# xuekt98/BBDM

Measured on NVIDIA H100. Metric: denoising-steps/sec (UNet fwd) at 256^2 pixel-BBDM, higher is better.
Workload: dtype bf16x3 (split-bf16 tensor-core products, fp32 accumulate: fp32-class)

## Files before the change

### bbdm_b200/csrc/conv_umma.cu

```cuda
#include "tc_common.cuh"
#include <stdlib.h>

namespace bbdm {

constexpr int UM_BM = 128;
constexpr int UM_BK = 64;
constexpr int UM_THREADS = 384;
constexpr int UM_PRODUCER_REGS = 40, UM_CONSUMER_REGS = 232;
static_assert(128 * UM_PRODUCER_REGS + 256 * UM_CONSUMER_REGS <= 65536, "conv_umma: register split");
constexpr int UM_SLICES = 4;

struct ConvParams {
  int B, H, W, Cout;
  int TW, TH, TB, tiles_w, tiles_h, tiles_b, n_tiles;
  int kb_per_tap;
  int K1;
  int K2;
  int taps;
  int up2;
  int origin;
  int w_per_image;
  int kb_per_chunk;
  const float* bias; const float* bias2;
  const float* residual; int res_mode;
  float* out; __nv_bfloat16* out_hi; __nv_bfloat16* out_lo;
  int out_nchw_c;
  float* stats;
  unsigned long long* fault;
};

template <int BN>
struct UmmaCfg {
  static constexpr uint32_t A_BYTES = UM_BM * UM_BK * 2;
  static constexpr uint32_t W_BYTES = BN * UM_BK * 2;
  static constexpr uint32_t STAGE3 = 2 * A_BYTES + 2 * W_BYTES;
  static constexpr uint32_t STAGE1 = A_BYTES + W_BYTES;
  static constexpr uint32_t SMEM_BUDGET = 200 * 1024;
  static constexpr int STAGES3 = (SMEM_BUDGET / STAGE3) > 6 ? 6 : (SMEM_BUDGET / STAGE3);
  static constexpr int STAGES1 = (SMEM_BUDGET / STAGE1) > 8 ? 8 : (SMEM_BUDGET / STAGE1);
};

template <int BN, bool F16>
__device__ __forceinline__ void conv_mma(float* d, uint64_t da, uint64_t db) {
  if (F16) {
    if (BN == 128) wgmma_n128_f16<0>(d, da, db, 1u); else wgmma_n64_f16<0>(d, da, db, 1u);
  } else {
    if (BN == 128) wgmma_n128_bf16<0>(d, da, db, 1u); else wgmma_n64_bf16<0>(d, da, db, 1u);
  }
}

struct EpiTile {
  int nb, tw, th, tb, phase;
  int bb[2], hh[2], ww[2];
  bool valid[2];
  int64_t pix[2];
};

__device__ __forceinline__ EpiTile epi_tile(const ConvParams& p, int tile, int n_blocks, int warp, int lane) {
  EpiTile e;
  e.nb = tile % n_blocks;
  int mt = tile / n_blocks;
  e.phase = 0;
  if (p.up2) { e.phase = mt & 3; mt >>= 2; }
  e.tw = mt % p.tiles_w; mt /= p.tiles_w;
  e.th = mt % p.tiles_h;
  e.tb = mt / p.tiles_h;
  const int OH = p.up2 ? 2 * p.H : p.H, OW = p.up2 ? 2 * p.W : p.W;
#pragma unroll
  for (int ri = 0; ri < 2; ++ri) {
    const int row = 16 * warp + (lane >> 2) + 8 * ri;
    const int ws = e.tw * p.TW + row % p.TW;
    const int hs = e.th * p.TH + (row / p.TW) % p.TH;
    e.bb[ri] = e.tb * p.TB + row / (p.TW * p.TH);
    e.valid[ri] = ws < p.W && hs < p.H && e.bb[ri] < p.B;
    e.hh[ri] = p.up2 ? 2 * hs + (e.phase >> 1) : hs;
    e.ww[ri] = p.up2 ? 2 * ws + (e.phase & 1) : ws;
    e.pix[ri] = ((int64_t)e.bb[ri] * OH + e.hh[ri]) * OW + e.ww[ri];
  }
  return e;
}

template <int BN>
__device__ __forceinline__ void epi_slice(const ConvParams& p, const float* racc, EpiTile e, int s, int warp,
                                          int lane, float (*stats_s)[BN][2]) {
  constexpr int JS = BN / 8 / UM_SLICES;
  if (e.nb * BN + s * (BN / UM_SLICES) >= p.Cout) return;
  asm volatile("" : "+r"(e.nb), "+r"(e.bb[0]), "+r"(e.bb[1]), "+r"(e.hh[0]), "+r"(e.hh[1]), "+r"(e.ww[0]),
               "+r"(e.ww[1]), "+l"(e.pix[0]), "+l"(e.pix[1]));
  const int OH = p.up2 ? 2 * p.H : p.H, OW = p.up2 ? 2 * p.W : p.W;
  const int n0 = e.nb * BN + 2 * (lane & 3);
  float2 v[2][JS];
#pragma unroll
  for (int ri = 0; ri < 2; ++ri) {
#pragma unroll
    for (int j = 0; j < JS; ++j) {
      const int jj = JS * s + j;
      const int nc = n0 + 8 * jj;
      v[ri][j] = make_float2(racc[4 * jj + 2 * ri], racc[4 * jj + 2 * ri + 1]);
      if (p.bias) { const float2 b = *reinterpret_cast<const float2*>(p.bias + nc); v[ri][j].x += b.x; v[ri][j].y += b.y; }
      if (p.bias2) { const float2 b = *reinterpret_cast<const float2*>(p.bias2 + nc); v[ri][j].x += b.x; v[ri][j].y += b.y; }
    }
  }
  if (p.res_mode == BBDM_RES_SAME || p.res_mode == BBDM_RES_UP2) {
#pragma unroll
    for (int ri = 0; ri < 2; ++ri) {
      if (!e.valid[ri]) continue;
      const int64_t rpix = p.res_mode == BBDM_RES_SAME
                               ? e.pix[ri]
                               : ((int64_t)e.bb[ri] * (OH >> 1) + (e.hh[ri] >> 1)) * (OW >> 1) + (e.ww[ri] >> 1);
      const float* rp = p.residual + rpix * p.Cout + n0 + 8 * JS * s;
#pragma unroll
      for (int j = 0; j < JS; ++j) {
        const float2 t = *reinterpret_cast<const float2*>(rp + 8 * j);
        v[ri][j].x += t.x; v[ri][j].y += t.y;
      }
    }
  } else if (p.res_mode == BBDM_RES_DOWN2) {
    const int64_t W2 = (int64_t)OW * 2;
#pragma unroll
    for (int ri = 0; ri < 2; ++ri) {
      if (!e.valid[ri]) continue;
      const float* rp0 = p.residual + (((int64_t)e.bb[ri] * OH * 2 + e.hh[ri] * 2) * W2 + e.ww[ri] * 2) * p.Cout +
                         n0 + 8 * JS * s;
#pragma unroll
      for (int j = 0; j < JS; ++j) {
        const float* rp = rp0 + 8 * j;
        const float2 t0 = *reinterpret_cast<const float2*>(rp), t1 = *reinterpret_cast<const float2*>(rp + p.Cout);
        const float2 t2 = *reinterpret_cast<const float2*>(rp + W2 * p.Cout);
        const float2 t3 = *reinterpret_cast<const float2*>(rp + (W2 + 1) * p.Cout);
        v[ri][j].x += 0.25f * (((t0.x + t1.x) + t2.x) + t3.x);
        v[ri][j].y += 0.25f * (((t0.y + t1.y) + t2.y) + t3.y);
      }
    }
  }
  float ssum[2 * JS], ssq[2 * JS];
#pragma unroll
  for (int j = 0; j < 2 * JS; ++j) { ssum[j] = 0.f; ssq[j] = 0.f; }
#pragma unroll
  for (int ri = 0; ri < 2; ++ri) {
    if (!e.valid[ri]) continue;
    const int bb = e.bb[ri], hh = e.hh[ri], ww = e.ww[ri];
    const int64_t pix = e.pix[ri];
#pragma unroll
    for (int j = 0; j < JS; ++j) {
      const int nc = n0 + 8 * (JS * s + j);
      const float2 w = v[ri][j];
      if (p.out_nchw_c > 0) {
        if (nc < p.out_nchw_c) p.out[(((int64_t)bb * p.out_nchw_c + nc) * OH + hh) * OW + ww] = w.x;
        if (nc + 1 < p.out_nchw_c) p.out[(((int64_t)bb * p.out_nchw_c + nc + 1) * OH + hh) * OW + ww] = w.y;
      } else if (p.out) {
        *reinterpret_cast<float2*>(p.out + pix * p.Cout + nc) = w;
      }
      if (p.out_hi) {
        uint32_t h, l;
        split2x(w.x, w.y, h, l);
        *reinterpret_cast<uint32_t*>(p.out_hi + pix * p.Cout + nc) = h;
        *reinterpret_cast<uint32_t*>(p.out_lo + pix * p.Cout + nc) = l;
      }
      ssum[2 * j] += w.x; ssq[2 * j] += w.x * w.x;
      ssum[2 * j + 1] += w.y; ssq[2 * j + 1] += w.y * w.y;
    }
  }
  if (p.stats) {
#pragma unroll
    for (int j = 0; j < 2 * JS; ++j) {
#pragma unroll
      for (int off = 4; off < 32; off <<= 1) {
        ssum[j] += __shfl_xor_sync(0xffffffffu, ssum[j], off);
        ssq[j] += __shfl_xor_sync(0xffffffffu, ssq[j], off);
      }
    }
    if (lane < 4) {
#pragma unroll
      for (int j = 0; j < 2 * JS; ++j) {
        const int c = 8 * (JS * s + (j >> 1)) + 2 * lane + (j & 1);
        stats_s[warp][c][0] = ssum[j];
        stats_s[warp][c][1] = ssq[j];
      }
    }
  }
}

template <int BN>
__device__ __forceinline__ void epi_stats_out(const ConvParams& p, const EpiTile& e, float (*stats_s)[BN][2]) {
  if (!p.stats) return;
  asm volatile("bar.sync 1, 256;" ::: "memory");
  const int64_t tile_lin =
      (((int64_t)e.tb * p.tiles_w * p.tiles_h + e.th * p.tiles_w + e.tw) * (p.up2 ? 4 : 1) + e.phase) * 4;
  int i0 = threadIdx.x;
  asm volatile("" : "+r"(i0));
  for (int i = i0; i < 4 * BN; i += 256) {
    const int q = i / BN, c = i % BN;
    if (e.nb * BN + c >= p.Cout) continue;
    const float s = stats_s[2 * q][c][0] + stats_s[2 * q + 1][c][0];
    const float sq = stats_s[2 * q][c][1] + stats_s[2 * q + 1][c][1];
    *reinterpret_cast<float2*>(p.stats + ((tile_lin + q) * p.Cout + e.nb * BN + c) * 2) = make_float2(s, sq);
  }
  asm volatile("bar.sync 1, 256;" ::: "memory");
}

template <int BN>
__device__ __forceinline__ void epi_slices(const ConvParams& p, const float* racc, const EpiTile& e, int s_begin,
                                           int s_end, int warp, int lane, float (*stats_s)[BN][2]) {
#pragma unroll
  for (int s = 0; s < UM_SLICES; ++s)
    if (s >= s_begin && s < s_end) epi_slice<BN>(p, racc, e, s, warp, lane, stats_s);
}

template <int BN, int PASSES, bool F16>
__global__ void __launch_bounds__(UM_THREADS, 1)
conv_umma_kernel(const __grid_constant__ CUtensorMap map_a_hi, const __grid_constant__ CUtensorMap map_a_lo,
                 const __grid_constant__ CUtensorMap map_w_hi, const __grid_constant__ CUtensorMap map_w_lo,
                 const __grid_constant__ CUtensorMap map_a2_hi, const __grid_constant__ CUtensorMap map_a2_lo,
                 const __grid_constant__ CUtensorMap map_w2_hi, const __grid_constant__ CUtensorMap map_w2_lo,
                 const ConvParams p) {
  using Cfg = UmmaCfg<BN>;
  constexpr int STAGES = PASSES == 3 ? Cfg::STAGES3 : Cfg::STAGES1;
  constexpr uint32_t STAGE_BYTES = PASSES == 3 ? Cfg::STAGE3 : Cfg::STAGE1;
  constexpr uint32_t OFF_ALO = Cfg::A_BYTES;
  constexpr uint32_t OFF_WHI = PASSES == 3 ? 2 * Cfg::A_BYTES : Cfg::A_BYTES;
  constexpr uint32_t OFF_WLO = OFF_WHI + Cfg::W_BYTES;
  constexpr int NR = BN / 2;
  static_assert(STAGES >= 2, "need at least a double buffer");

  extern __shared__ uint8_t smem_raw[];
  __shared__ __align__(8) uint64_t bars[2 * 8];
  __shared__ int abort_s;
  __shared__ __align__(16) float stats_s[8][BN][2];

  const uint32_t tiles_base = (smem_u32(smem_raw) + 1023u) & ~1023u;
  const int warp = threadIdx.x >> 5, lane = threadIdx.x & 31;
  const uint32_t bar_full = smem_u32(&bars[0]);
  const uint32_t bar_empty = smem_u32(&bars[8]);
  volatile int* abort_flag = &abort_s;

  if (threadIdx.x == 0) {
    abort_s = 0;
    for (int i = 0; i < STAGES; ++i) { mbar_init(bar_full + 8 * i, 1); mbar_init(bar_empty + 8 * i, 8); }
    asm volatile("fence.mbarrier_init.release.cluster;" ::: "memory");
  }
  __syncthreads();

  const int n_blocks = (p.Cout + BN - 1) / BN;
  const int total_tiles = p.n_tiles * n_blocks * (p.up2 ? 4 : 1);
  const int KB = p.K1 + p.K2;

  if (warp >= 8) {
    setmaxnreg_dec<UM_PRODUCER_REGS>();
    if (warp == 8 && lane == 0) {
      int stage = 0;
      uint32_t phase_bit = 0;
      for (int tile = blockIdx.x; tile < total_tiles; tile += gridDim.x) {
        const int nb = tile % n_blocks;
        int mt = tile / n_blocks;
        int phase = 0;
        if (p.up2) { phase = mt & 3; mt >>= 2; }
        const int tw = mt % p.tiles_w; mt /= p.tiles_w;
        const int th = mt % p.tiles_h;
        const int tb = mt / p.tiles_h;
        const int w0 = tw * p.TW, h0 = th * p.TH, b0 = tb * p.TB, n0 = nb * BN;
        for (int kb = 0; kb < KB; ++kb) {
          mbar_wait(bar_empty + 8 * stage, phase_bit ^ 1, abort_flag, p.fault, 0xE0000000ull | (unsigned)kb);
          const uint32_t sbase = tiles_base + stage * STAGE_BYTES;
          const uint32_t full = bar_full + 8 * stage;
          mbar_expect_tx(full, STAGE_BYTES);
          if (kb < p.K1) {
            const int tap = kb / p.kb_per_tap, cb = kb - tap * p.kb_per_tap;
            int dy = 0, dx = 0, wtap = tap;
            if (p.up2) {
              const int r = tap >> 1, c = tap & 1;
              dy = (phase >> 1) ? r : r - 1;
              dx = (phase & 1) ? c : c - 1;
              wtap = phase * 4 + tap;
            } else if (p.taps == 9) { dy = tap / 3 - 1; dx = tap % 3 - 1; }
            else if (p.taps == 4) { dy = (tap >> 1) + p.origin; dx = (tap & 1) + p.origin; }
            else if (p.w_per_image) wtap = tb;
            tma_load_4d(sbase, &map_a_hi, full, cb * UM_BK, w0 + dx, h0 + dy, b0);
            if (PASSES == 3) tma_load_4d(sbase + OFF_ALO, &map_a_lo, full, cb * UM_BK, w0 + dx, h0 + dy, b0);
            tma_load_3d(sbase + OFF_WHI, &map_w_hi, full, cb * UM_BK, n0, wtap);
            if (PASSES == 3) tma_load_3d(sbase + OFF_WLO, &map_w_lo, full, cb * UM_BK, n0, wtap);
          } else {
            const int cb = kb - p.K1;
            tma_load_4d(sbase, &map_a2_hi, full, cb * UM_BK, w0, h0, b0);
            if (PASSES == 3) tma_load_4d(sbase + OFF_ALO, &map_a2_lo, full, cb * UM_BK, w0, h0, b0);
            tma_load_3d(sbase + OFF_WHI, &map_w2_hi, full, cb * UM_BK, n0, 0);
            if (PASSES == 3) tma_load_3d(sbase + OFF_WLO, &map_w2_lo, full, cb * UM_BK, n0, 0);
          }
          if (++stage == STAGES) { stage = 0; phase_bit ^= 1; }
        }
      }
    }
    return;
  }

  setmaxnreg_inc<UM_CONSUMER_REGS>();
  const int wg = warp >> 2;
  const uint32_t a_off = (uint32_t)wg * 64 * 128;
  int stage = 0;
  uint32_t phase_bit = 0;
  float racc[NR];
  EpiTile pend;
  bool pending = false;
  int slice = 0;
  for (int tile = blockIdx.x; tile < total_tiles; tile += gridDim.x) {
    for (int kb0 = 0; kb0 < KB; kb0 += p.kb_per_chunk) {
      const int kb1 = kb0 + p.kb_per_chunk < KB ? kb0 + p.kb_per_chunk : KB;
      float acc[NR];
#pragma unroll
      for (int j = 0; j < NR; ++j) acc[j] = 0.f;
      int prev = -1;
      for (int kb = kb0; kb < kb1; ++kb) {
        mbar_wait(bar_full + 8 * stage, phase_bit, abort_flag, p.fault, 0xF0000000ull | (unsigned)kb);
        const uint32_t sbase = tiles_base + stage * STAGE_BYTES;
        const uint64_t da_hi = make_sw128_desc(sbase + a_off);
        const uint64_t da_lo = make_sw128_desc(sbase + OFF_ALO + a_off);
        const uint64_t db_hi = make_sw128_desc(sbase + OFF_WHI);
        const uint64_t db_lo = make_sw128_desc(sbase + OFF_WLO);
        wgmma_fence();
#pragma unroll
        for (int k = 0; k < UM_BK / 16; ++k) {
          const uint64_t ko = (uint64_t)(k * 32 >> 4);
          if (PASSES == 3) {
            conv_mma<BN, F16>(acc, da_lo + ko, db_hi + ko);
            conv_mma<BN, F16>(acc, da_hi + ko, db_lo + ko);
          }
          conv_mma<BN, F16>(acc, da_hi + ko, db_hi + ko);
        }
        wgmma_commit();
        wgmma_wait<1>();
        if (prev >= 0 && lane == 0) mbar_arrive(bar_empty + 8 * prev);
        prev = stage;
        if (++stage == STAGES) { stage = 0; phase_bit ^= 1; }
        if (pending) {
          const int s_end = kb + 1 < kb1 ? slice + 1 : UM_SLICES;
          epi_slices<BN>(p, racc, pend, slice, s_end, warp, lane, stats_s);
          slice = s_end;
        }
      }
      if (pending) {
        epi_stats_out<BN>(p, pend, stats_s);
        pending = false;
      }
      wgmma_wait<0>();
      reg_fence<NR>(acc);
      if (lane == 0) mbar_arrive(bar_empty + 8 * prev);
      if (kb0 == 0) {
#pragma unroll
        for (int j = 0; j < NR; ++j) racc[j] = 0.f + acc[j];
      } else {
#pragma unroll
        for (int j = 0; j < NR; ++j) racc[j] += acc[j];
      }
    }
    pend = epi_tile(p, tile, n_blocks, warp, lane);
    pending = true;
    slice = 0;
  }
  if (pending) {
    epi_slices<BN>(p, racc, pend, 0, UM_SLICES, warp, lane, stats_s);
    epi_stats_out<BN>(p, pend, stats_s);
  }
}

static int make_act_map(CUtensorMap* m, const void* ptr, int B, int H, int W, int C, int TW, int TH, int TB,
                        bool f16) {
  EncodeTiledFn enc = get_encode();
  BBDM_REQUIRE(enc != nullptr, "cuTensorMapEncodeTiled entry point not available");
  cuuint64_t dims[4] = {(cuuint64_t)C, (cuuint64_t)W, (cuuint64_t)H, (cuuint64_t)B};
  cuuint64_t strides[3] = {(cuuint64_t)C * 2, (cuuint64_t)W * C * 2, (cuuint64_t)H * W * C * 2};
  cuuint32_t box[4] = {(cuuint32_t)UM_BK, (cuuint32_t)TW, (cuuint32_t)TH, (cuuint32_t)TB};
  cuuint32_t es[4] = {1, 1, 1, 1};
  CUresult r = enc(m, f16 ? CU_TENSOR_MAP_DATA_TYPE_FLOAT16 : CU_TENSOR_MAP_DATA_TYPE_BFLOAT16, 4, const_cast<void*>(ptr), dims, strides, box, es,
                   CU_TENSOR_MAP_INTERLEAVE_NONE, CU_TENSOR_MAP_SWIZZLE_128B, CU_TENSOR_MAP_L2_PROMOTION_L2_256B,
                   CU_TENSOR_MAP_FLOAT_OOB_FILL_NONE);
  BBDM_REQUIRE(r == CUDA_SUCCESS, "cuTensorMapEncodeTiled(activation) failed: %d (B=%d H=%d W=%d C=%d box=%dx%dx%d)",
               (int)r, B, H, W, C, TW, TH, TB);
  return BBDM_OK;
}

static int make_w_map(CUtensorMap* m, const void* ptr, int taps, int Cout, int Cin, int BN, bool f16) {
  EncodeTiledFn enc = get_encode();
  BBDM_REQUIRE(enc != nullptr, "cuTensorMapEncodeTiled entry point not available");
  cuuint64_t dims[3] = {(cuuint64_t)Cin, (cuuint64_t)Cout, (cuuint64_t)taps};
  cuuint64_t strides[2] = {(cuuint64_t)Cin * 2, (cuuint64_t)Cout * Cin * 2};
  cuuint32_t box[3] = {(cuuint32_t)UM_BK, (cuuint32_t)BN, 1};
  cuuint32_t es[3] = {1, 1, 1};
  CUresult r = enc(m, f16 ? CU_TENSOR_MAP_DATA_TYPE_FLOAT16 : CU_TENSOR_MAP_DATA_TYPE_BFLOAT16, 3, const_cast<void*>(ptr), dims, strides, box, es,
                   CU_TENSOR_MAP_INTERLEAVE_NONE, CU_TENSOR_MAP_SWIZZLE_128B, CU_TENSOR_MAP_L2_PROMOTION_L2_256B,
                   CU_TENSOR_MAP_FLOAT_OOB_FILL_NONE);
  BBDM_REQUIRE(r == CUDA_SUCCESS, "cuTensorMapEncodeTiled(weight) failed: %d (taps=%d Cout=%d Cin=%d BN=%d)", (int)r,
               taps, Cout, Cin, BN);
  return BBDM_OK;
}

static int pow2_floor(int x) { int p = 1; while (p * 2 <= x) p *= 2; return p; }
static int pow2_ceil(int x) { int p = 1; while (p < x) p *= 2; return p; }

template <int BN, int PASSES, bool F16>
static int launch_conv(const CUtensorMap* maps, const ConvParams& p, int grid, cudaStream_t s) {
  using Cfg = UmmaCfg<BN>;
  constexpr int STAGES = PASSES == 3 ? Cfg::STAGES3 : Cfg::STAGES1;
  constexpr uint32_t STAGE_BYTES = PASSES == 3 ? Cfg::STAGE3 : Cfg::STAGE1;
  const size_t smem = (size_t)STAGES * STAGE_BYTES + 1024;
  static DeviceOnce configured;
  if (configured.need()) {
    BBDM_CUDA_CHECK(cudaFuncSetAttribute(conv_umma_kernel<BN, PASSES, F16>, cudaFuncAttributeMaxDynamicSharedMemorySize, (int)smem));
    configured.mark();
  }
  conv_umma_kernel<BN, PASSES, F16><<<grid, UM_THREADS, smem, s>>>(maps[0], maps[1], maps[2], maps[3], maps[4], maps[5],
                                                                  maps[6], maps[7], p);
  BBDM_LAUNCH_CHECK();
  return BBDM_OK;
}

}

using namespace bbdm;

static void tile_geometry(int H, int W, int* TW, int* TH, int* TB) {
  *TW = pow2_floor(W) < 16 ? pow2_floor(W) : 16;
  const int th = pow2_ceil(H);
  *TH = th < UM_BM / *TW ? th : UM_BM / *TW;
  *TB = UM_BM / (*TW * *TH);
}

extern "C" int bbdm_conv_umma_geometry(int H, int W, int* TW, int* TH, int* TB, int* rows_per_image) {
  BBDM_REQUIRE(H > 0 && W >= 4, "conv_umma_geometry: need H > 0, W >= 4");
  int tw, th, tb;
  tile_geometry(H, W, &tw, &th, &tb);
  if (TW) *TW = tw;
  if (TH) *TH = th;
  if (TB) *TB = tb;
  if (rows_per_image) *rows_per_image = tb == 1 ? 4 * ((W + tw - 1) / tw) * ((H + th - 1) / th) : 0;
  return BBDM_OK;
}

extern "C" int bbdm_conv_umma(const BbdmConvArgs* a, void* stream) {
  BBDM_REQUIRE(a != nullptr, "conv_umma: null args");
  BBDM_REQUIRE(a->B > 0 && a->H > 0 && a->W > 0, "conv_umma: bad spatial shape");
  BBDM_REQUIRE(a->taps == 1 || a->taps == 9 || a->taps == 4, "conv_umma: taps must be 1, 4 or 9 (got %d)", a->taps);
  BBDM_REQUIRE(!a->upsample2x || (a->taps == 4 && a->Cin2 == 0), "conv_umma: upsample2x needs the 16 phase taps and no fused 1x1");
  BBDM_REQUIRE(a->Cin > 0 && a->Cin % 32 == 0, "conv_umma: Cin %% 32 != 0 (Cin=%d)", a->Cin);
  BBDM_REQUIRE(a->Cout > 0 && a->Cout % 32 == 0, "conv_umma: Cout %% 32 != 0 (Cout=%d)", a->Cout);
  BBDM_REQUIRE(a->Cin2 >= 0 && a->Cin2 % 32 == 0, "conv_umma: Cin2 %% 32 != 0 (Cin2=%d)", a->Cin2);
  BBDM_REQUIRE(a->passes == 1 || a->passes == 3, "conv_umma: passes must be 1 or 3");
  BBDM_REQUIRE(a->a_hi && a->w_hi && (a->passes == 1 || (a->a_lo && a->w_lo)), "conv_umma: missing operand plane");
  if (a->Cin2) BBDM_REQUIRE(a->a2_hi && a->w2_hi && (a->passes == 1 || (a->a2_lo && a->w2_lo)), "conv_umma: missing 1x1 operand plane");
  BBDM_REQUIRE(a->out || (a->out_hi && a->out_lo), "conv_umma: no output");
  BBDM_REQUIRE((a->out_hi == nullptr) == (a->out_lo == nullptr), "conv_umma: out hi/lo must come in pairs");
  BBDM_REQUIRE(a->res_mode >= 0 && a->res_mode <= 3 && (a->res_mode == 0 || a->residual), "conv_umma: bad residual");
  if (a->res_mode == BBDM_RES_UP2 && !a->upsample2x) BBDM_REQUIRE(a->H % 2 == 0 && a->W % 2 == 0, "conv_umma: RES_UP2 needs even H, W");
  BBDM_REQUIRE(a->W >= 4, "conv_umma: W < 4 not supported (use conv_direct)");
  BBDM_REQUIRE(a->window_origin == 0 || a->window_origin == -1, "conv_umma: window_origin must be 0 or -1 (got %d)",
               a->window_origin);
  BBDM_REQUIRE(a->window_origin == 0 || (a->taps == 4 && !a->upsample2x),
               "conv_umma: window_origin -1 needs taps == 4 and no upsample2x");
  const bool wpi = a->weights_per_image != 0, f16 = a->operand_f16 != 0;
  if (wpi) BBDM_REQUIRE(a->taps == 1 && a->Cin2 == 0 && !a->upsample2x, "conv_umma: weights_per_image needs taps == 1 and no fused operand");
  if (wpi) BBDM_REQUIRE(a->Cin % 64 == 0 && a->Cout % 64 == 0, "conv_umma: weights_per_image needs Cin, Cout %% 64 == 0");

  ConvParams p;
  p.B = a->B; p.H = a->H; p.W = a->W; p.Cout = a->Cout;
  tile_geometry(a->H, a->W, &p.TW, &p.TH, &p.TB);
  p.tiles_w = (a->W + p.TW - 1) / p.TW;
  p.tiles_h = (a->H + p.TH - 1) / p.TH;
  p.tiles_b = (a->B + p.TB - 1) / p.TB;
  p.n_tiles = p.tiles_w * p.tiles_h * p.tiles_b;
  int BN = (a->Cout + 127) / 128 * 128 == (a->Cout + 63) / 64 * 64 ? 128 : 64;
  {
    const int64_t m_tiles = (int64_t)p.n_tiles * (a->upsample2x ? 4 : 1);
    const int64_t want = (int64_t)(0.7 * num_sms());
    if (BN > 64 && m_tiles * ((a->Cout + BN - 1) / BN) < want) BN = 64;
  }
  p.kb_per_tap = (a->Cin + UM_BK - 1) / UM_BK;
  p.K1 = a->taps * p.kb_per_tap;
  p.K2 = (a->Cin2 + UM_BK - 1) / UM_BK;
  p.taps = a->taps;
  p.up2 = a->upsample2x ? 1 : 0;
  p.origin = a->window_origin;
  p.w_per_image = wpi ? 1 : 0;
  static int wino_chunk = -1;
  if (wino_chunk < 0) { const char* e = getenv("BBDM_WINO_CHUNK"); wino_chunk = (e && atoi(e) > 0) ? atoi(e) : 0; }
  const int wchunk = wino_chunk ? wino_chunk : (a->Cin >= 512 ? 4 : 2);
  p.kb_per_chunk = wpi ? wchunk : (a->passes == 3 ? 4 : 8);
  if (wpi) BBDM_REQUIRE(p.TB == 1, "conv_umma: weights_per_image needs 128-pixel tiles inside one image (H*W >= 128)");
  p.bias = a->bias; p.bias2 = a->Cin2 ? a->bias2 : nullptr;
  p.residual = a->residual; p.res_mode = a->res_mode;
  p.out = a->out; p.out_hi = (__nv_bfloat16*)a->out_hi; p.out_lo = (__nv_bfloat16*)a->out_lo;
  p.out_nchw_c = a->out_nchw_channels;
  p.stats = a->stats_partial;
  BBDM_REQUIRE(p.out_nchw_c >= 0 && p.out_nchw_c <= a->Cout && (p.out_nchw_c == 0 || (a->out && !a->out_hi)),
               "conv_umma: bad out_nchw_channels");
  p.fault = device_fault_ptr();
  BBDM_REQUIRE(p.fault != nullptr, "conv_umma: device fault word unavailable");

  BBDM_REQUIRE(p.stats == nullptr || (p.TB == 1 && p.out_nchw_c == 0),
               "conv_umma: stats_partial needs a tile inside one image (H*W >= 128) and NHWC output");
  CUtensorMap maps[8];
  int rc;
  if ((rc = make_act_map(&maps[0], a->a_hi, a->B, a->H, a->W, a->Cin, p.TW, p.TH, p.TB, f16))) return rc;
  if ((rc = make_act_map(&maps[1], a->passes == 3 ? a->a_lo : a->a_hi, a->B, a->H, a->W, a->Cin, p.TW, p.TH, p.TB, f16))) return rc;
  const int wtaps = a->upsample2x ? 16 : (wpi ? a->B : a->taps);
  if ((rc = make_w_map(&maps[2], a->w_hi, wtaps, a->Cout, a->Cin, BN, f16))) return rc;
  if ((rc = make_w_map(&maps[3], a->passes == 3 ? a->w_lo : a->w_hi, wtaps, a->Cout, a->Cin, BN, f16))) return rc;
  if (a->Cin2) {
    if ((rc = make_act_map(&maps[4], a->a2_hi, a->B, a->H, a->W, a->Cin2, p.TW, p.TH, p.TB, f16))) return rc;
    if ((rc = make_act_map(&maps[5], a->passes == 3 ? a->a2_lo : a->a2_hi, a->B, a->H, a->W, a->Cin2, p.TW, p.TH, p.TB, f16))) return rc;
    if ((rc = make_w_map(&maps[6], a->w2_hi, 1, a->Cout, a->Cin2, BN, f16))) return rc;
    if ((rc = make_w_map(&maps[7], a->passes == 3 ? a->w2_lo : a->w2_hi, 1, a->Cout, a->Cin2, BN, f16))) return rc;
  } else {
    maps[4] = maps[0]; maps[5] = maps[1]; maps[6] = maps[2]; maps[7] = maps[3];
  }
  const int64_t total = (int64_t)p.n_tiles * ((a->Cout + BN - 1) / BN) * (p.up2 ? 4 : 1);
  BBDM_REQUIRE(total < (1ll << 30), "conv_umma: too many tiles");
  const int grid = (int)(total < num_sms() ? total : num_sms());
  cudaStream_t s = (cudaStream_t)stream;
  const bool p3 = a->passes == 3;
  if (BN == 128) {
    if (f16) return p3 ? launch_conv<128, 3, true>(maps, p, grid, s) : launch_conv<128, 1, true>(maps, p, grid, s);
    return p3 ? launch_conv<128, 3, false>(maps, p, grid, s) : launch_conv<128, 1, false>(maps, p, grid, s);
  }
  if (f16) return p3 ? launch_conv<64, 3, true>(maps, p, grid, s) : launch_conv<64, 1, true>(maps, p, grid, s);
  return p3 ? launch_conv<64, 3, false>(maps, p, grid, s) : launch_conv<64, 1, false>(maps, p, grid, s);
}
```

Measured before the change: 6.081.

## Ping-pong accumulators across chunks to keep wgmma in flight between chunk boundaries

For the 3-pass (split-bf16) path, the consumer now alternates between two accumulator register sets. The next chunk's first k-block is issued before the previous chunk's accumulator is drained and promoted, so the pipeline no longer stalls on wgmma_wait<0> at every chunk boundary. The epilogue is recomputed per slice using a rolled loop to limit register pressure. The 1-pass path keeps the old structure, and the epilogue slice helper now takes pre-picked values. The cost is a doubled accumulator register footprint, which risks spills given the 232-register consumer budget.

```diff
diff --git a/bbdm_b200/csrc/conv_umma.cu b/bbdm_b200/csrc/conv_umma.cu
--- a/bbdm_b200/csrc/conv_umma.cu
+++ b/bbdm_b200/csrc/conv_umma.cu
@@ -81,22 +81,19 @@
 }
 
 template <int BN>
-__device__ __forceinline__ void epi_slice(const ConvParams& p, const float* racc, EpiTile e, int s, int warp,
-                                          int lane, float (*stats_s)[BN][2]) {
+__device__ __forceinline__ void epi_slice(const ConvParams& p, float2 (&v)[2][BN / 8 / UM_SLICES], EpiTile e, int s,
+                                          int warp, int lane, float (*stats_s)[BN][2]) {
   constexpr int JS = BN / 8 / UM_SLICES;
   if (e.nb * BN + s * (BN / UM_SLICES) >= p.Cout) return;
   asm volatile("" : "+r"(e.nb), "+r"(e.bb[0]), "+r"(e.bb[1]), "+r"(e.hh[0]), "+r"(e.hh[1]), "+r"(e.ww[0]),
                "+r"(e.ww[1]), "+l"(e.pix[0]), "+l"(e.pix[1]));
   const int OH = p.up2 ? 2 * p.H : p.H, OW = p.up2 ? 2 * p.W : p.W;
   const int n0 = e.nb * BN + 2 * (lane & 3);
-  float2 v[2][JS];
 #pragma unroll
   for (int ri = 0; ri < 2; ++ri) {
 #pragma unroll
     for (int j = 0; j < JS; ++j) {
-      const int jj = JS * s + j;
-      const int nc = n0 + 8 * jj;
-      v[ri][j] = make_float2(racc[4 * jj + 2 * ri], racc[4 * jj + 2 * ri + 1]);
+      const int nc = n0 + 8 * (JS * s + j);
       if (p.bias) { const float2 b = *reinterpret_cast<const float2*>(p.bias + nc); v[ri][j].x += b.x; v[ri][j].y += b.y; }
       if (p.bias2) { const float2 b = *reinterpret_cast<const float2*>(p.bias2 + nc); v[ri][j].x += b.x; v[ri][j].y += b.y; }
     }
@@ -199,12 +196,37 @@
   asm volatile("bar.sync 1, 256;" ::: "memory");
 }
 
-template <int BN>
+template <int BN, bool ROLLED>
 __device__ __forceinline__ void epi_slices(const ConvParams& p, const float* racc, const EpiTile& e, int s_begin,
                                            int s_end, int warp, int lane, float (*stats_s)[BN][2]) {
-#pragma unroll
-  for (int s = 0; s < UM_SLICES; ++s)
-    if (s >= s_begin && s < s_end) epi_slice<BN>(p, racc, e, s, warp, lane, stats_s);
+  constexpr int JS = BN / 8 / UM_SLICES;
+  auto pick = [&](float2 (&v)[2][JS], int t) {
+#pragma unroll
+    for (int ri = 0; ri < 2; ++ri)
+#pragma unroll
+      for (int j = 0; j < JS; ++j) {
+        const int jj = JS * t + j;
+        v[ri][j] = make_float2(racc[4 * jj + 2 * ri], racc[4 * jj + 2 * ri + 1]);
+      }
+  };
+  if constexpr (ROLLED) {
+#pragma unroll 1
+    for (int s = s_begin; s < s_end; ++s) {
+      float2 v[2][JS];
+#pragma unroll
+      for (int t = 0; t < UM_SLICES; ++t)
+        if (t == s) pick(v, t);
+      epi_slice<BN>(p, v, e, s, warp, lane, stats_s);
+    }
+  } else {
+#pragma unroll
+    for (int s = 0; s < UM_SLICES; ++s)
+      if (s >= s_begin && s < s_end) {
+        float2 v[2][JS];
+        pick(v, s);
+        epi_slice<BN>(p, v, e, s, warp, lane, stats_s);
+      }
+  }
 }
 
 template <int BN, int PASSES, bool F16>
@@ -298,67 +320,143 @@
   const uint32_t a_off = (uint32_t)wg * 64 * 128;
   int stage = 0;
   uint32_t phase_bit = 0;
+  if constexpr (PASSES == 1) {
+    float racc[NR];
+    EpiTile pend;
+    bool pending = false;
+    int slice = 0;
+    for (int tile = blockIdx.x; tile < total_tiles; tile += gridDim.x) {
+      for (int kb0 = 0; kb0 < KB; kb0 += p.kb_per_chunk) {
+        const int kb1 = kb0 + p.kb_per_chunk < KB ? kb0 + p.kb_per_chunk : KB;
+        float acc[NR];
+#pragma unroll
+        for (int j = 0; j < NR; ++j) acc[j] = 0.f;
+        int prev = -1;
+        for (int kb = kb0; kb < kb1; ++kb) {
+          mbar_wait(bar_full + 8 * stage, phase_bit, abort_flag, p.fault, 0xF0000000ull | (unsigned)kb);
+          const uint32_t sbase = tiles_base + stage * STAGE_BYTES;
+          wgmma_fence();
+#pragma unroll
+          for (int k = 0; k < UM_BK / 16; ++k) {
+            const uint64_t ko = (uint64_t)(k * 32 >> 4);
+            conv_mma<BN, F16>(acc, make_sw128_desc(sbase + a_off) + ko, make_sw128_desc(sbase + OFF_WHI) + ko);
+          }
+          wgmma_commit();
+          wgmma_wait<1>();
+          if (prev >= 0 && lane == 0) mbar_arrive(bar_empty + 8 * prev);
+          prev = stage;
+          if (++stage == STAGES) { stage = 0; phase_bit ^= 1; }
+          if (pending) {
+            const int s_end = kb + 1 < kb1 ? slice + 1 : UM_SLICES;
+            epi_slices<BN, false>(p, racc, pend, slice, s_end, warp, lane, stats_s);
+            slice = s_end;
+          }
+        }
+        if (pending) {
+          epi_stats_out<BN>(p, pend, stats_s);
+          pending = false;
+        }
+        wgmma_wait<0>();
+        reg_fence<NR>(acc);
+        if (lane == 0) mbar_arrive(bar_empty + 8 * prev);
+        if (kb0 == 0) {
+#pragma unroll
+          for (int j = 0; j < NR; ++j) racc[j] = 0.f + acc[j];
+        } else {
+#pragma unroll
+          for (int j = 0; j < NR; ++j) racc[j] += acc[j];
+        }
+      }
+      pend = epi_tile(p, tile, n_blocks, warp, lane);
+      pending = true;
+      slice = 0;
+    }
+    if (pending) {
+      epi_slices<BN, false>(p, racc, pend, 0, UM_SLICES, warp, lane, stats_s);
+      epi_stats_out<BN>(p, pend, stats_s);
+    }
+    return;
+  }
+
+  int prev = -1;
   float racc[NR];
-  EpiTile pend;
-  bool pending = false;
-  int slice = 0;
-  for (int tile = blockIdx.x; tile < total_tiles; tile += gridDim.x) {
-    for (int kb0 = 0; kb0 < KB; kb0 += p.kb_per_chunk) {
-      const int kb1 = kb0 + p.kb_per_chunk < KB ? kb0 + p.kb_per_chunk : KB;
-      float acc[NR];
-#pragma unroll
-      for (int j = 0; j < NR; ++j) acc[j] = 0.f;
-      int prev = -1;
-      for (int kb = kb0; kb < kb1; ++kb) {
-        mbar_wait(bar_full + 8 * stage, phase_bit, abort_flag, p.fault, 0xF0000000ull | (unsigned)kb);
-        const uint32_t sbase = tiles_base + stage * STAGE_BYTES;
-        const uint64_t da_hi = make_sw128_desc(sbase + a_off);
-        const uint64_t da_lo = make_sw128_desc(sbase + OFF_ALO + a_off);
-        const uint64_t db_hi = make_sw128_desc(sbase + OFF_WHI);
-        const uint64_t db_lo = make_sw128_desc(sbase + OFF_WLO);
-        wgmma_fence();
-#pragma unroll
-        for (int k = 0; k < UM_BK / 16; ++k) {
-          const uint64_t ko = (uint64_t)(k * 32 >> 4);
-          if (PASSES == 3) {
-            conv_mma<BN, F16>(acc, da_lo + ko, db_hi + ko);
-            conv_mma<BN, F16>(acc, da_hi + ko, db_lo + ko);
-          }
-          conv_mma<BN, F16>(acc, da_hi + ko, db_hi + ko);
-        }
-        wgmma_commit();
-        wgmma_wait<1>();
-        if (prev >= 0 && lane == 0) mbar_arrive(bar_empty + 8 * prev);
-        prev = stage;
-        if (++stage == STAGES) { stage = 0; phase_bit ^= 1; }
-        if (pending) {
-          const int s_end = kb + 1 < kb1 ? slice + 1 : UM_SLICES;
-          epi_slices<BN>(p, racc, pend, slice, s_end, warp, lane, stats_s);
-          slice = s_end;
-        }
-      }
-      if (pending) {
-        epi_stats_out<BN>(p, pend, stats_s);
-        pending = false;
-      }
-      wgmma_wait<0>();
-      reg_fence<NR>(acc);
-      if (lane == 0) mbar_arrive(bar_empty + 8 * prev);
-      if (kb0 == 0) {
-#pragma unroll
-        for (int j = 0; j < NR; ++j) racc[j] = 0.f + acc[j];
-      } else {
-#pragma unroll
-        for (int j = 0; j < NR; ++j) racc[j] += acc[j];
-      }
-    }
-    pend = epi_tile(p, tile, n_blocks, warp, lane);
-    pending = true;
-    slice = 0;
-  }
-  if (pending) {
-    epi_slices<BN>(p, racc, pend, 0, UM_SLICES, warp, lane, stats_s);
-    epi_stats_out<BN>(p, pend, stats_s);
+  float acc0[NR], acc1[NR];
+  int fl_tile = -1;
+  bool fl_first = false, fl_last = false;
+
+  auto promote = [&](float (&fl)[NR]) {
+    reg_fence<NR>(fl);
+    if (fl_first) {
+#pragma unroll
+      for (int j = 0; j < NR; ++j) racc[j] = 0.f + fl[j];
+    } else {
+#pragma unroll
+      for (int j = 0; j < NR; ++j) racc[j] += fl[j];
+    }
+  };
+  auto kblock = [&](float (&acc)[NR], int kb) {
+    mbar_wait(bar_full + 8 * stage, phase_bit, abort_flag, p.fault, 0xF0000000ull | (unsigned)kb);
+    const uint32_t sbase = tiles_base + stage * STAGE_BYTES;
+    const uint64_t da_hi = make_sw128_desc(sbase + a_off);
+    const uint64_t da_lo = make_sw128_desc(sbase + OFF_ALO + a_off);
+    const uint64_t db_hi = make_sw128_desc(sbase + OFF_WHI);
+    const uint64_t db_lo = make_sw128_desc(sbase + OFF_WLO);
+    wgmma_fence();
+#pragma unroll
+    for (int k = 0; k < UM_BK / 16; ++k) {
+      const uint64_t ko = (uint64_t)(k * 32 >> 4);
+      conv_mma<BN, F16>(acc, da_lo + ko, db_hi + ko);
+      conv_mma<BN, F16>(acc, da_hi + ko, db_lo + ko);
+      conv_mma<BN, F16>(acc, da_hi + ko, db_hi + ko);
+    }
+    wgmma_commit();
+    wgmma_wait<1>();
+    if (prev >= 0 && lane == 0) mbar_arrive(bar_empty + 8 * prev);
+    prev = stage;
+    if (++stage == STAGES) { stage = 0; phase_bit ^= 1; }
+  };
+  int tile = blockIdx.x, kb0 = 0;
+  auto chunk = [&](float (&acc)[NR], float (&fl)[NR]) {
+    const int kb1 = kb0 + p.kb_per_chunk < KB ? kb0 + p.kb_per_chunk : KB;
+    const bool epi = fl_tile >= 0 && fl_last;
+    int slice = 0;
+    auto epi_step = [&](int kb) {
+      if (!epi) return;
+      const int s_end = kb + 1 < kb1 ? slice + 1 : UM_SLICES;
+      epi_slices<BN, true>(p, racc, epi_tile(p, fl_tile, n_blocks, warp, lane), slice, s_end, warp, lane, stats_s);
+      slice = s_end;
+    };
+#pragma unroll
+    for (int j = 0; j < NR; ++j) acc[j] = 0.f;
+    kblock(acc, kb0);
+    if (fl_tile >= 0) promote(fl);
+    for (int kb = kb0;;) {
+      epi_step(kb);
+      if (++kb == kb1) break;
+      kblock(acc, kb);
+    }
+    if (epi) epi_stats_out<BN>(p, epi_tile(p, fl_tile, n_blocks, warp, lane), stats_s);
+    fl_tile = tile;
+    fl_first = kb0 == 0;
+    fl_last = kb1 == KB;
+    kb0 = kb1;
+    if (kb0 == KB) { kb0 = 0; tile += gridDim.x; }
+  };
+  auto finish = [&](float (&fl)[NR]) {
+    if (fl_tile < 0) return;
+    wgmma_wait<0>();
+    if (lane == 0) mbar_arrive(bar_empty + 8 * prev);
+    promote(fl);
+    const EpiTile e = epi_tile(p, fl_tile, n_blocks, warp, lane);
+    epi_slices<BN, true>(p, racc, e, 0, UM_SLICES, warp, lane, stats_s);
+    epi_stats_out<BN>(p, e, stats_s);
+  };
+
+  for (;;) {
+    if (tile >= total_tiles) { finish(acc1); break; }
+    chunk(acc0, acc1);
+    if (tile >= total_tiles) { finish(acc0); break; }
+    chunk(acc1, acc0);
   }
 }
 
```

After: 6.148, median of 6. 1.1% higher.
